# ElusAegis/metal-msm-gpu-acceleration

Hardware: AMD Instinct MI355X
Metric: BN254 G1 MSM/s at log_size=20 (5 instances) (higher is better)
Workload: dtype u32x8 (256-bit Montgomery integer)

## Files before the change

### include/msm_amd.h

```cpp
#ifndef MSM_AMD_H
#define MSM_AMD_H

#include <stddef.h>
#include <stdint.h>

#ifdef __cplusplus
extern "C" {
#endif

typedef struct msm_amd_ctx msm_amd_ctx;

enum {
  MSM_AMD_OK = 0,
  MSM_AMD_DEVICE_NOT_FOUND = 1,
  MSM_AMD_LIBRARY_ERROR = 2,
  MSM_AMD_FUNCTION_ERROR = 3,
  MSM_AMD_PIPELINE_ERROR = 4,
  MSM_AMD_INPUT_ERROR = 5,
  MSM_AMD_FILE_OPEN_ERROR = 6,
  MSM_AMD_DESERIALIZATION_ERROR = 7,
  MSM_AMD_INVALID_DATA = 8
};

enum {
// ... 150 lines not shown
size_t msm_amd_instances_default_path(const char* dir, uint32_t log_size, uint32_t num_instances, char* buf,
                                      size_t buf_len);
int msm_amd_to_wire(int scalar_layout, int point_layout, const void* scalars, const void* points, size_t n,
                    void* scalars_be32_out, void* points_be32_out);
int msm_amd_from_wire(int scalar_layout, int point_layout, const void* scalars_be32, const void* points_be32,
                      size_t n, void* scalars_out, void* points_out);

int msm_amd_prepare_buckets_indices(msm_amd_ctx* ctx, const uint32_t* scalars_be32, size_t n, uint32_t window_size,
                                    uint32_t num_windows, uint32_t* pairs_out);
int msm_amd_sort_buckets_indices(msm_amd_ctx* ctx, uint32_t* pairs, size_t n_pairs);
int msm_amd_sort_pairs_device(msm_amd_ctx* ctx, void* d_pairs, size_t n_pairs, uint32_t key_bits, float* kernel_ms);
int msm_amd_bucket_wise_accumulation(msm_amd_ctx* ctx, const uint32_t* sorted_pairs, size_t n_pairs,
                                     const uint32_t* points_be32, size_t n_points, uint32_t total_buckets,
                                     uint32_t* buckets_out);
int msm_amd_sum_reduction(msm_amd_ctx* ctx, const uint32_t* buckets_be32, uint32_t buckets_size,
                          uint32_t num_windows, uint32_t* res_out);
int msm_amd_final_accumulation(const uint32_t* res_be32, uint32_t num_windows, uint32_t window_size,
                               uint32_t* point_out);

enum {
  MSM_AMD_OP_UINT_ADD = 0,
  MSM_AMD_OP_UINT_SUB = 1,
  MSM_AMD_OP_UINT_PROD = 2,
  MSM_AMD_OP_UINT_SHL = 3,
  MSM_AMD_OP_UINT_SHR = 4,
  MSM_AMD_OP_FP_ADD = 5,
  MSM_AMD_OP_FP_SUB = 6,
  MSM_AMD_OP_FP_MUL = 7,
  MSM_AMD_OP_FP_NEG = 8,
  MSM_AMD_OP_FP_POW = 9,
  MSM_AMD_OP_EC_ADD = 10,
  MSM_AMD_OP_EC_MUL = 11,
  MSM_AMD_OP_EC_MADD = 12,
  MSM_AMD_OP_EC_DBL = 13,
  MSM_AMD_OP_FP29_MUL = 14,
  MSM_AMD_OP_FP29_SQR = 15,
  MSM_AMD_OP_FP29_SUB_K4E30 = 16,
  MSM_AMD_OP_FP29_SUB_K8E30 = 17,
  MSM_AMD_OP_FP29_SUB_K8E31 = 18,
  MSM_AMD_OP_FP29_SUB_K16E30 = 19,
  MSM_AMD_OP_FP29_SUB_K16E31 = 20,
  MSM_AMD_OP_FP29_ROUNDTRIP = 21,
  MSM_AMD_OP_EC29_MADD = 22,
  MSM_AMD_OP_EC29_ADD = 23,
  MSM_AMD_OP_EC29_MADD_CHAIN = 24,
  MSM_AMD_OP_EC29_ADD_CHAIN = 25,
  MSM_AMD_OP_EC29_MMADD = 26,
  MSM_AMD_OP_H64_FP_MUL = 27,
  MSM_AMD_OP_H64_FP_ADD = 28,
  MSM_AMD_OP_H64_FP_SUB = 29,
  MSM_AMD_OP_H64_EC_ADD = 30,
  MSM_AMD_OP_H64_EC_DBL = 31,
  MSM_AMD_OP_FP29_MUL_KARATSUBA = 32,
  MSM_AMD_OP_FP29_LOCKSTEP_PAIR = 33,
  MSM_AMD_OP_FP29_LOCKSTEP_MIX = 34,
  MSM_AMD_OP_FP29_LOCKSTEP_TRIPLE = 35,
  MSM_AMD_OP_FP29_MUL2_KARATSUBA = 36,
  MSM_AMD_OP_H64_FP_INV = 37,
  MSM_AMD_OP_H64_FP_INV_FERMAT = 38
};
int msm_amd_test_op(msm_amd_ctx* ctx, int op, const uint32_t* a, const uint32_t* b, uint32_t* out, size_t count);
int msm_amd_test_op_host(int op, const uint32_t* a, const uint32_t* b, uint32_t* out, size_t count);

enum {
  MSM_AMD_RAW_FE_MUL = 0,
  MSM_AMD_RAW_FE_SQR = 1,
  MSM_AMD_RAW_FE_MUL2 = 2,
  MSM_AMD_RAW_FE_SUB_K4E30 = 3,
  MSM_AMD_RAW_FE_SUB_K8E30 = 4,
  MSM_AMD_RAW_FE_SUB_K8E31 = 5,
  MSM_AMD_RAW_FE_SUB_K16E30 = 6,
  MSM_AMD_RAW_FE_SUB_K16E31 = 7,
  MSM_AMD_RAW_FE_NORM = 8,
  MSM_AMD_RAW_FE_NEG = 9,
  MSM_AMD_RAW_FE_NEG_WIDE = 10,
  MSM_AMD_RAW_FE_CANONICAL = 11,
  MSM_AMD_RAW_FE_TO_EXT = 12,
  MSM_AMD_RAW_FE_PACK_UNPACK = 13,
  MSM_AMD_RAW_FE_ZERO = 14,
  MSM_AMD_RAW_PT_MADD = 15,
  MSM_AMD_RAW_PT_MMADD = 16,
  MSM_AMD_RAW_PT_ADD_NZ = 17,
  MSM_AMD_RAW_PT_ADD = 18,
  MSM_AMD_RAW_PT_DOUBLE = 19
};
int msm_amd_test_op_raw(msm_amd_ctx* ctx, int op, const uint32_t* a, const uint32_t* b, uint32_t* out, size_t count);
int msm_amd_test_op_raw_host(int op, const uint32_t* a, const uint32_t* b, uint32_t* out, size_t count);

int msm_amd_test_hold(msm_amd_ctx* ctx, uint32_t max_ms, void** handle);
int msm_amd_test_release(msm_amd_ctx* ctx, void* handle);

enum {
  MSM_AMD_TP_C = 0, MSM_AMD_TP_W, MSM_AMD_TP_W_DIGITS, MSM_AMD_TP_N, MSM_AMD_TP_N_SCALARS, MSM_AMD_TP_LB, MSM_AMD_TP_NB,
  MSM_AMD_TP_CH, MSM_AMD_TP_HB, MSM_AMD_TP_MB, MSM_AMD_TP_FB, MSM_AMD_TP_Q, MSM_AMD_TP_TILED, MSM_AMD_TP_BALLOT,
  MSM_AMD_TP_WIDE_DIGITS, MSM_AMD_TP_LONE,
  MSM_AMD_TP_TOTAL_ITEMS, MSM_AMD_TP_MULTI_COUNT, MSM_AMD_TP_DEFERRED,
  MSM_AMD_TP_RED_GROUP, MSM_AMD_TP_RB_THREADS, MSM_AMD_TP_INSTANCES, MSM_AMD_TP_WORKSPACE, MSM_AMD_TP_FRONT_THREADS,
  MSM_AMD_TEST_PLAN_WORDS
};
int msm_amd_test_last_plan(msm_amd_ctx* ctx, uint32_t j, uint32_t* out, size_t count);
enum {
  MSM_AMD_STAGE_DIGITS = 0,
  MSM_AMD_STAGE_SORTED = 1,
  MSM_AMD_STAGE_BUCKET_SIZE = 2,
  MSM_AMD_STAGE_BUCKET_START = 3,
  MSM_AMD_STAGE_ITEM_START = 4,
  MSM_AMD_STAGE_WIN_ITEMS = 5,
  MSM_AMD_STAGE_ORDER = 6,
  MSM_AMD_STAGE_MULTI_LIST = 7,
  MSM_AMD_STAGE_BUCKETS = 8,
  MSM_AMD_STAGE_PARTIAL = 9
};
int msm_amd_test_stage_copy(msm_amd_ctx* ctx, uint32_t j, int which, void* out, size_t* bytes);
int msm_amd_test_fill_workspaces(msm_amd_ctx* ctx, uint8_t byte);

int msm_amd_last_timings(const msm_amd_ctx* ctx, msm_amd_timings* out);
uint64_t msm_amd_algorithmic_bytes(size_t n, uint32_t window_size, int accumulate_only);
const char* msm_amd_version(void);

#ifdef __cplusplus
}
#endif
#endif
```

### metal-msm-gpu-acceleration_amd/__init__.py

```python
from __future__ import annotations

import ctypes
import os
from ctypes import POINTER, c_char_p, c_float, c_int, c_size_t, c_uint32, c_uint64, c_void_p

_HERE = os.path.dirname(os.path.abspath(__file__))
LIB_PATH = os.environ.get("MSM_AMD_LIB") or os.path.join(_HERE, "libmsm_amd.so")

(OK, DEVICE_NOT_FOUND, LIBRARY_ERROR, FUNCTION_ERROR, PIPELINE_ERROR, INPUT_ERROR, FILE_OPEN_ERROR,
 DESERIALIZATION_ERROR, INVALID_DATA) = range(9)
SCALAR_MONT_LE, SCALAR_CANON_LE, SCALAR_CANON_BE32 = 0, 1, 2
POINT_H2C_AFFINE, POINT_ARK_PROJECTIVE, POINT_ARK_AFFINE, POINT_JAC_BE32, POINT_PREPARED, POINT_TABLES = 0, 1, 2, 3, 4, 5
POINT_BYTES = {POINT_H2C_AFFINE: 64, POINT_ARK_PROJECTIVE: 96, POINT_ARK_AFFINE: 72, POINT_JAC_BE32: 96}
(OP_UINT_ADD, OP_UINT_SUB, OP_UINT_PROD, OP_UINT_SHL, OP_UINT_SHR, OP_FP_ADD, OP_FP_SUB, OP_FP_MUL, OP_FP_NEG,
 OP_FP_POW, OP_EC_ADD, OP_EC_MUL, OP_EC_MADD, OP_EC_DBL, OP_FP29_MUL, OP_FP29_SQR, OP_FP29_SUB_K4E30,
 OP_FP29_SUB_K8E30, OP_FP29_SUB_K8E31, OP_FP29_SUB_K16E30, OP_FP29_SUB_K16E31, OP_FP29_ROUNDTRIP, OP_EC29_MADD,
 OP_EC29_ADD, OP_EC29_MADD_CHAIN, OP_EC29_ADD_CHAIN, OP_EC29_MMADD, OP_H64_FP_MUL, OP_H64_FP_ADD, OP_H64_FP_SUB,
 OP_H64_EC_ADD, OP_H64_EC_DBL, OP_FP29_MUL_KARATSUBA, OP_FP29_LOCKSTEP_PAIR, OP_FP29_LOCKSTEP_MIX,
 OP_FP29_LOCKSTEP_TRIPLE, OP_FP29_MUL2_KARATSUBA, OP_H64_FP_INV, OP_H64_FP_INV_FERMAT) = range(39)
(RAW_FE_MUL, RAW_FE_SQR, RAW_FE_MUL2, RAW_FE_SUB_K4E30, RAW_FE_SUB_K8E30, RAW_FE_SUB_K8E31, RAW_FE_SUB_K16E30,
 RAW_FE_SUB_K16E31, RAW_FE_NORM, RAW_FE_NEG, RAW_FE_NEG_WIDE, RAW_FE_CANONICAL, RAW_FE_TO_EXT, RAW_FE_PACK_UNPACK,
 RAW_FE_ZERO, RAW_PT_MADD, RAW_PT_MMADD, RAW_PT_ADD_NZ, RAW_PT_ADD, RAW_PT_DOUBLE) = range(20)
RAW_IN_WORDS, RAW_OUT_WORDS = 36, 40


def op_is_point(op):
    return 10 <= op <= 13 or 22 <= op <= 26 or op in (OP_H64_EC_ADD, OP_H64_EC_DBL)

EXPORTS = [
    "msm_amd_init", "msm_amd_init_reusable", "msm_amd_get_global", "msm_amd_destroy", "msm_amd_strerror",
    "msm_amd_last_error", "msm_amd_set_window_size", "msm_amd_auto_window_size", "msm_amd_auto_window_size_lone", "msm_amd_gpu_msm_h2c",
    "msm_amd_gpu_msm_h2c_sync", "msm_amd_cpu_dispatch_below", "msm_amd_host_register", "msm_amd_host_unregister",
    "msm_amd_metal_msm_ark", "msm_amd_msm", "msm_amd_msm_batch", "msm_amd_msm_best", "msm_amd_gpu_with_cpu",
    "msm_amd_reference_split", "msm_amd_msm_device",
    "msm_amd_msm_batch_device", "msm_amd_submit_batch_device", "msm_amd_wait_batch", "msm_amd_device_alloc", "msm_amd_device_free", "msm_amd_copy_to_device",
    "msm_amd_copy_to_host", "msm_amd_stream", "msm_amd_synchronize", "msm_amd_generate_instance",
    "msm_amd_prepare_buckets_indices", "msm_amd_sort_buckets_indices", "msm_amd_bucket_wise_accumulation",
    "msm_amd_sum_reduction", "msm_amd_final_accumulation", "msm_amd_test_op", "msm_amd_test_op_host",
    "msm_amd_test_op_raw", "msm_amd_test_op_raw_host",
    "msm_amd_last_timings",
    "msm_amd_algorithmic_bytes", "msm_amd_version",
    "msm_amd_instances_save", "msm_amd_instances_open", "msm_amd_instances_count", "msm_amd_instances_size",
    "msm_amd_instances_read", "msm_amd_instances_close", "msm_amd_instances_default_path", "msm_amd_to_wire",
    "msm_amd_from_wire", "msm_amd_sort_pairs_device", "msm_amd_bases_upload", "msm_amd_bases_prepare_device",
    "msm_amd_msm_prepared", "msm_amd_sum_points", "msm_amd_tables_build", "msm_amd_tables_build_device",
    "msm_amd_tables_info", "msm_amd_tables_free", "msm_amd_msm_tables",
    "msm_amd_set_wait_timeout_ms", "msm_amd_set_bases_cache", "msm_amd_bases_cache_stats", "msm_amd_test_hold",
    "msm_amd_test_release", "msm_amd_msm_batch_multi", "msm_amd_msm_batch_multi_device", "msm_amd_msm_range_multi", "msm_amd_shard_range",
    "msm_amd_submit_batch_multi_device", "msm_amd_wait_batch_multi", "msm_amd_bases_cache_invalidate",
    "msm_amd_set_bases_cache_verify",
    "msm_amd_scalar_bytes", "msm_amd_point_bytes", "msm_amd_shard_owner",
    "msm_amd_shard_count", "msm_amd_ctx_device", "msm_amd_pin_thread_to_device", "msm_amd_gather_init",
    "msm_amd_gather_size", "msm_amd_gather_all", "msm_amd_gather_last_error", "msm_amd_gather_destroy",
    "msm_amd_host_msm", "msm_amd_tuned_split", "msm_amd_host_threads", "msm_amd_generate_instance_host", "msm_amd_test_op_ifma",
    "msm_amd_test_last_plan", "msm_amd_test_stage_copy", "msm_amd_test_fill_workspaces",
]

TEST_PLAN_FIELDS = ("c", "W", "W_digits", "n", "n_scalars", "lb", "nb", "CH", "hb", "mb", "fb", "Q", "tiled", "ballot",
                    "wide_digits", "lone", "total_items", "multi_count", "deferred", "red_group", "rb_threads",
                    "instances", "workspace", "front_threads")
(STAGE_DIGITS, STAGE_SORTED, STAGE_BUCKET_SIZE, STAGE_BUCKET_START, STAGE_ITEM_START, STAGE_WIN_ITEMS, STAGE_ORDER,
 STAGE_MULTI_LIST, STAGE_BUCKETS, STAGE_PARTIAL) = range(10)


AFTER_SORT_FN = ctypes.CFUNCTYPE(None, c_void_p)


class Timings(ctypes.Structure):
    _fields_ = [("convert_ms", c_float), ("digits_ms", c_float), ("sort_ms", c_float), ("accumulate_ms", c_float),
                ("reduce_ms", c_float), ("final_ms", c_float), ("total_gpu_ms", c_float), ("n", c_uint32),
                ("window_size", c_uint32), ("num_windows", c_uint32), ("reserved", c_uint32),
                ("accumulate_kernel_ms", c_float), ("reserved2", c_float * 3)]


class MsmError(RuntimeError):

    def __init__(self, status, detail=""):
        self.status = status
        super().__init__(f"msm_amd status {status}: {_lib().msm_amd_strerror(status).decode()} {detail}")


_LIB = None


def _lib():
    global _LIB
    if _LIB is None:
        if not os.path.exists(LIB_PATH):
            raise FileNotFoundError(f"{LIB_PATH} not built: run `python -c 'import __graft_entry__ as g; g.build()'`")
        L = ctypes.CDLL(LIB_PATH)
        L.msm_amd_strerror.restype = c_char_p
        L.msm_amd_strerror.argtypes = [c_int]
        L.msm_amd_last_error.restype = c_char_p
        L.msm_amd_last_error.argtypes = [c_void_p]
        L.msm_amd_version.restype = c_char_p
        L.msm_amd_init.argtypes = [c_int, POINTER(c_void_p)]
        L.msm_amd_bases_upload.argtypes = [c_void_p, c_int, c_void_p, c_size_t, POINTER(c_void_p)]
        L.msm_amd_bases_prepare_device.argtypes = [c_void_p, c_int, c_void_p, c_size_t, c_void_p]
        L.msm_amd_msm_prepared.argtypes = [c_void_p, c_int, c_void_p, c_void_p, c_size_t, c_void_p]
        L.msm_amd_tables_build.argtypes = [c_void_p, c_int, c_void_p, c_size_t, c_uint32, POINTER(c_void_p)]
        L.msm_amd_tables_build_device.argtypes = [c_void_p, c_int, c_void_p, c_size_t, c_uint32, POINTER(c_void_p)]
        L.msm_amd_tables_info.argtypes = [c_void_p, c_void_p, POINTER(c_size_t), POINTER(c_uint32), POINTER(c_uint32),
                                          POINTER(c_size_t)]
        L.msm_amd_tables_free.argtypes = [c_void_p, c_void_p]
        L.msm_amd_msm_tables.argtypes = [c_void_p, c_void_p, c_int, c_void_p, c_void_p]
# ... 580 lines not shown
```

### metal-msm-gpu-acceleration_amd/csrc/bn254_ec29.hip.h

```cpp
#pragma once
#include "bn254_ec.hip.h"
#include "bn254_fq29.hip.h"

namespace msm_amd {

struct AffI {
  fe29 x, y;
};
struct AffPacked {
  u256 x, y;
};
struct PtI {
  fe29 x, y, zz, zzz;
};
static_assert(sizeof(AffPacked) == 64, "AffPacked must be 64 bytes");
static_assert(sizeof(PtI) == 144, "PtI must be 144 bytes");

MSM_HD bool affi_is_identity(const AffI& p) {
  uint32_t o = 0;
  MSM_UNROLL for (int i = 0; i < 9; ++i) o |= p.x.l[i] | p.y.l[i];
  return o == 0;
}
MSM_HD bool pti_is_identity(const PtI& p) { return Fq29::is_zero_limbs(p.zz); }

// ... 149 lines not shown
  const fe29 Pp = pin_limbs(P), Rp = pin_limbs(R), X1 = pin_limbs(px), Y1 = pin_limbs(py);
  const fe29 PP = Fq29::sqr_np(Pp);
  const fe29 PPP = Fq29::mul_np(Pp, PP);
  const fe29 Q = Fq29::mul_np(X1, PP);
  const fe29 RR = Fq29::sqr_np(Rp);
  PtI r;
  r.x = Fq29::norm(Fq29::sub<K8E31>(RR, Fq29::add(PPP, Fq29::add(Q, Q))));
  const fe29 T = Fq29::norm(Fq29::sub<K16E30>(Q, r.x));
  r.y = Fq29::mul2_np(Rp, T, Y1, Fq29::neg_wide(PPP));
  r.zz = PP;
  r.zzz = PPP;
  return r;
}

MSM_HD PtI pti_madd(const PtI& p, const AffI& q, bool& vanished) {
#if defined(MSM_AMD_EXPERIMENTS) && defined(MSM_FQ29_LOCKSTEP)
  fe29 U2, S2;
  Fq29::mul_pair(q.x, p.zz, q.y, p.zzz, U2, S2);
#elif defined(MSM_AMD_EXPERIMENTS) && defined(MSM_FQ29_KARATSUBA)
  const fe29 U2 = Fq29::mul_karatsuba(q.x, p.zz);
  const fe29 S2 = Fq29::mul_karatsuba(q.y, p.zzz);
#else
  fe29 U2, S2;
  PtI pp = p;
  pti_madd_head(pp, q.x, q.y, U2, S2);
  return pti_madd_tail(pp, U2, S2, [&]() { return q; }, vanished);
#endif
#if defined(MSM_AMD_EXPERIMENTS) && (defined(MSM_FQ29_LOCKSTEP) || defined(MSM_FQ29_KARATSUBA))
  const fe29 P = Fq29::norm(Fq29::sub<K16E30>(U2, p.x));
  const fe29 R = Fq29::norm(Fq29::sub<K8E30>(S2, p.y));
  if (Fq29::maybe_zero(P, 18)) {
    MSM_ISA_MARK("rare mixed_addition");
    if (Fq29::is_zero_exact(P)) {
      if (Fq29::is_zero_exact(R)) return pti_double(pti_from_affi(q));
      vanished = true;
      return pti_identity();
    }
  }
  MSM_ISA_MARK("resume mixed_addition");
  PtI r;
#if defined(MSM_AMD_EXPERIMENTS) && defined(MSM_FQ29_LOCKSTEP)
  fe29 PP, RR, PPP, Q;
  Fq29::sqr_pair(P, R, PP, RR);
  Fq29::mul_triple(P, PP, p.x, PP, p.zz, PP, PPP, Q, r.zz);
  r.x = Fq29::norm(Fq29::sub<K8E31>(RR, Fq29::add(PPP, Fq29::add(Q, Q))));
  const fe29 T = Fq29::sub<K16E30>(Q, r.x);
  Fq29::mul2_mul_pair(R, T, p.y, Fq29::neg_wide(PPP), p.zzz, PPP, r.y, r.zzz);
#elif defined(MSM_AMD_EXPERIMENTS) && defined(MSM_FQ29_KARATSUBA)
  const fe29 PP = Fq29::sqr(P);
  const fe29 PPP = Fq29::mul_karatsuba(P, PP);
  const fe29 Q = Fq29::mul_karatsuba(p.x, PP);
  const fe29 RR = Fq29::sqr(R);
  r.x = Fq29::norm(Fq29::sub<K8E31>(RR, Fq29::add(PPP, Fq29::add(Q, Q))));
  const fe29 T = Fq29::sub<K16E30>(Q, r.x);
  r.y = Fq29::mul2_karatsuba_second(R, T, p.y, Fq29::neg_wide(PPP));
  r.zz = Fq29::mul_karatsuba(p.zz, PP);
  r.zzz = Fq29::mul_karatsuba(p.zzz, PPP);
#endif
  return r;
#endif
}

MSM_HD PtI pti_mmadd(const fe29& px, const fe29& py, const AffI& q, bool& vanished) {
  fe29 P, R;
  pti_mmadd_head(px, py, q.x, q.y, P, R);
  return pti_mmadd_tail(px, py, P, R, [&]() { return q; }, vanished);
}


#if defined(MSM_AMD_EXPERIMENTS)
#include "experiments/ec29_variants.inc"
#endif

MSM_HD PtI pti_madd(const PtI& p, const AffI& q) {
  bool vanished = false;
  return pti_madd(p, q, vanished);
}
MSM_HD PtI pti_mmadd(const fe29& px, const fe29& py, const AffI& q) {
  bool vanished = false;
  return pti_mmadd(px, py, q, vanished);
}

MSM_HD PtI pti_add_nz(const PtI& p_in, const PtI& q_in, bool& vanished) {
  PtI p, q;
  p.x = pin_limbs(p_in.x); p.y = pin_limbs(p_in.y); p.zz = pin_limbs(p_in.zz); p.zzz = pin_limbs(p_in.zzz);
  q.x = pin_limbs(q_in.x); q.y = pin_limbs(q_in.y); q.zz = pin_limbs(q_in.zz); q.zzz = pin_limbs(q_in.zzz);
  const fe29 U1a = Fq29::mul_np(p.x, q.zz);
  const fe29 U2 = Fq29::mul_np(q.x, p.zz);
  const fe29 S1a = Fq29::mul_np(p.y, q.zzz);
  const fe29 S2 = Fq29::mul_np(q.y, p.zzz);
  const fe29 P0 = Fq29::norm(Fq29::sub<K4E30>(U2, U1a));
  const fe29 R0 = Fq29::norm(Fq29::sub<K4E30>(S2, S1a));
  if (Fq29::maybe_zero(P0, 6)) {
    if (Fq29::is_zero_exact(P0)) {
      if (Fq29::is_zero_exact(R0)) return pti_double(p);
      vanished = true;
      return pti_identity();
    }
  }
  const fe29 P = pin_limbs(P0), R = pin_limbs(R0), U1 = pin_limbs(U1a), S1 = pin_limbs(S1a), ZZ1 = pin_limbs(p.zz),
             ZZ2 = pin_limbs(q.zz), ZZZ1 = pin_limbs(p.zzz), ZZZ2 = pin_limbs(q.zzz);
  const fe29 PP = Fq29::sqr_np(P);
  const fe29 PPP = Fq29::mul_np(P, PP);
  const fe29 Q = Fq29::mul_np(U1, PP);
  const fe29 RR = Fq29::sqr_np(R);
  PtI r;
  r.x = Fq29::norm(Fq29::sub<K8E31>(RR, Fq29::add(PPP, Fq29::add(Q, Q))));
  const fe29 T = Fq29::sub<K16E30>(Q, r.x);
  r.y = Fq29::mul2_np(R, T, S1, Fq29::neg_wide(PPP));
  r.zz = Fq29::mul_np(Fq29::mul_np(ZZ1, ZZ2), PP);
  r.zzz = Fq29::mul_np(Fq29::mul_np(ZZZ1, ZZZ2), PPP);
  return r;
}
MSM_HD PtI pti_add_nz(const PtI& p, const PtI& q) {
  bool vanished = false;
  return pti_add_nz(p, q, vanished);
}

MSM_HD PtI pti_add(const PtI& p, const PtI& q) {
  if (pti_is_identity(p)) return q;
  if (pti_is_identity(q)) return p;
  return pti_add_nz(p, q);
}

}
```

### metal-msm-gpu-acceleration_amd/csrc/bn254_fq29.hip.h

```cpp
#pragma once
#include "bn254_fq.hip.h"

namespace msm_amd {

struct fe29 {
  uint32_t l[9];
};

MSM_HD uint32_t limb32(uint32_t x) {
#if defined(__HIP_DEVICE_COMPILE__) && !defined(MSM_FQ29_NOPIN)
  asm("" : "+v"(x));
#endif
  return x;
}
MSM_HD fe29 pin_limbs(const fe29& a) {
  fe29 r;
#if defined(__HIP_DEVICE_COMPILE__)
  _Pragma("unroll") for (int i = 0; i < 9; ++i) r.l[i] = limb32(a.l[i]);
#else
  r = a;
#endif
  return r;
}

#if defined(__HIP_DEVICE_COMPILE__)
#define MSM_ISA_MARK(name) asm volatile("; MSM_MARK " name)
#else
#define MSM_ISA_MARK(name) ((void)0)
#endif

enum KSel { K4E30 = 0, K8E30 = 1, K8E31 = 2, K16E30 = 3, K16E31 = 4 };

struct Fq29 {
  static constexpr uint32_t MASK = 0x1FFFFFFFu;
  static constexpr uint32_t INV = 0x04866389u;
  static constexpr uint32_t PINV = 0x1B799C77u;

  MSM_HD static constexpr uint32_t p(int i) {
    constexpr uint32_t c[9] = {0x187CFD47u, 0x010460B6u, 0x1C72A34Fu, 0x02D522D0u, 0x1585D978u,
                               0x02DB40C0u, 0x00A6E141u, 0x0E5C2634u, 0x0030644Eu};
    return c[i];
  }
  MSM_HD static constexpr uint32_t one_c(int i) {
    constexpr uint32_t c[9] = {0x157CCC21u, 0x141C2758u, 0x185230D3u, 0x014C0419u, 0x0AA36FB9u,
                               0x1D4240CEu, 0x11D54C07u, 0x052AC7A8u, 0x000DC836u};
    return c[i];
  }
  MSM_HD static constexpr uint32_t cin_c(int i) {
    constexpr uint32_t c[9] = {0x13349CA1u, 0x1A5D84A8u, 0x0A3E5CACu, 0x100249E0u, 0x12B951E8u,
                               0x0E92D304u, 0x14CB95B3u, 0x041B9D3Du, 0x00058003u};
    return c[i];
  }
  MSM_HD static constexpr uint32_t dout_c(int i) {
    constexpr uint32_t c[9] = {0x058F0D9Du, 0x1AEA1C6Eu, 0x11C2CF74u, 0x11D651EBu, 0x1462C0A7u,
                               0x11B7BC3Cu, 0x1CBD99BAu, 0x183340FBu, 0x000E0A77u};
    return c[i];
  }
  MSM_HD static constexpr uint32_t kc(int sel, int i) {
    constexpr uint32_t c[5][9] = {
        {0x41F3F51Cu, 0x441182D9u, 0x51CA8D3Au, 0x4B548B41u, 0x561765DEu, 0x4B6D0300u, 0x429B8502u, 0x597098CEu, 0x00C19137u},
        {0x43E7EA38u, 0x482305B4u, 0x43951A76u, 0x56A91685u, 0x4C2ECBBEu, 0x56DA0603u, 0x45370A06u, 0x52E1319Eu, 0x01832271u},
        {0x83E7EA38u, 0x882305B2u, 0x83951A74u, 0x96A91683u, 0x8C2ECBBCu, 0x96DA0601u, 0x85370A04u, 0x92E1319Cu, 0x0183226Fu},
        {0x47CFD470u, 0x50460B6Au, 0x472A34EEu, 0x4D522D0Cu, 0x585D977Fu, 0x4DB40C08u, 0x4A6E140Fu, 0x45C2633Eu, 0x030644E5u},
        {0x87CFD470u, 0x90460B68u, 0x872A34ECu, 0x8D522D0Au, 0x985D977Du, 0x8DB40C06u, 0x8A6E140Du, 0x85C2633Cu, 0x030644E3u}};
    return c[sel][i];
  }

  MSM_HD static fe29 zero() {
    fe29 r;
    MSM_UNROLL for (int i = 0; i < 9; ++i) r.l[i] = 0;
    return r;
  }
  MSM_HD static fe29 one() {
    fe29 r;
    MSM_UNROLL for (int i = 0; i < 9; ++i) r.l[i] = one_c(i);
    return r;
  }
  MSM_HD static bool is_zero_limbs(const fe29& a) {
    uint32_t o = 0;
    MSM_UNROLL for (int i = 0; i < 9; ++i) o |= a.l[i];
    return o == 0;
  }

  MSM_HD static fe29 add(const fe29& a, const fe29& b) {
    fe29 r;
    MSM_UNROLL for (int i = 0; i < 9; ++i) r.l[i] = a.l[i] + b.l[i];
    return r;
  }

  template <int SEL>
  MSM_HD static fe29 sub(const fe29& a, const fe29& b) {
    fe29 r;
    MSM_UNROLL for (int i = 0; i < 9; ++i) r.l[i] = (a.l[i] + kc(SEL, i)) - b.l[i];
    return r;
  }

  MSM_HD static fe29 neg(const fe29& a) { return norm(sub<K4E30>(zero(), a)); }
  MSM_HD static fe29 neg_wide(const fe29& a) { return sub<K4E30>(zero(), a); }

  MSM_HD static fe29 norm(const fe29& a) {
    fe29 r;
    r.l[0] = a.l[0] & MASK;
    MSM_UNROLL for (int i = 1; i < 8; ++i) r.l[i] = (a.l[i] & MASK) + (a.l[i - 1] >> 29);
    r.l[8] = a.l[8] + (a.l[7] >> 29);
    return r;
  }

  MSM_HD static fe29 reduce_columns(uint64_t (&A)[17]) {
    uint64_t carry = 0;
    MSM_UNROLL for (int k = 0; k < 9; ++k) {
      A[k] += carry;
      const uint32_t m = ((uint32_t)A[k] * INV) & MASK;
      MSM_UNROLL for (int j = 0; j < 9; ++j) A[k + j] += (uint64_t)m * p(j);
      carry = A[k] >> 29;
    }
    fe29 r;
    MSM_UNROLL for (int k = 9; k < 17; ++k) {
      A[k] += carry;
      r.l[k - 9] = (uint32_t)A[k] & MASK;
      carry = A[k] >> 29;
    }
    r.l[8] = (uint32_t)carry;
    return r;
  }


#if defined(MSM_AMD_EXPERIMENTS)
#include "experiments/fq29_variants.inc"
#endif

  template <bool PIN = true>
  MSM_HD static fe29 mul(const fe29& a_in, const fe29& b_in) {
    const fe29 a = PIN ? pin_limbs(a_in) : a_in, b = PIN ? pin_limbs(b_in) : b_in;
#if defined(MSM_AMD_EXPERIMENTS) && defined(MSM_FQ29_FIPS)
    {
      const fe29* const xs[1] = {&a};
      const fe29* const ys[1] = {&b};
      return fips<1>(xs, ys);
    }
#endif
    uint64_t A[17];
    MSM_UNROLL for (int k = 0; k < 17; ++k) {
      uint64_t s = 0;
      MSM_UNROLL for (int i = 0; i < 9; ++i) {
        const int j = k - i;
        if (j >= 0 && j < 9) s += (uint64_t)a.l[i] * b.l[j];
      }
      A[k] = s;
    }
    return reduce_columns(A);
  }

  template <bool PIN = true>
  MSM_HD static fe29 mul2(const fe29& a_in, const fe29& b_in, const fe29& c_in, const fe29& d_in) {
    const fe29 a = PIN ? pin_limbs(a_in) : a_in, b = PIN ? pin_limbs(b_in) : b_in, c = PIN ? pin_limbs(c_in) : c_in,
               d = PIN ? pin_limbs(d_in) : d_in;
#if defined(MSM_AMD_EXPERIMENTS) && defined(MSM_FQ29_FIPS)
    {
      const fe29* const xs[2] = {&a, &c};
      const fe29* const ys[2] = {&b, &d};
      return fips<2>(xs, ys);
    }
#endif
    uint64_t A[17];
    MSM_UNROLL for (int k = 0; k < 17; ++k) {
      uint64_t s = 0;
      MSM_UNROLL for (int i = 0; i < 9; ++i) {
        const int j = k - i;
        if (j >= 0 && j < 9) {
          s += (uint64_t)a.l[i] * b.l[j];
          s += (uint64_t)c.l[i] * d.l[j];
        }
      }
      A[k] = s;
    }
    return reduce_columns(A);
  }

  template <bool PIN = true>
  MSM_HD static fe29 sqr(const fe29& a_in) {
    const fe29 a = PIN ? pin_limbs(a_in) : a_in;
#if defined(MSM_AMD_EXPERIMENTS) && defined(MSM_FQ29_FIPS)
    {
      fe29 d2;
      MSM_UNROLL for (int i = 0; i < 9; ++i) d2.l[i] = a.l[i] << 1;
      const fe29* const xs[1] = {&d2};
      const fe29* const ys[1] = {&a};
      return fips<1, true>(xs, ys);
    }
#endif
    uint32_t d[9];
    MSM_UNROLL for (int i = 0; i < 9; ++i) d[i] = a.l[i] << 1;
    uint64_t A[17];
    MSM_UNROLL for (int k = 0; k < 17; ++k) {
      uint64_t s = 0;
      MSM_UNROLL for (int i = 0; i < 9; ++i) {
        const int j = k - i;
        if (j >= 0 && j < 9 && i < j) s += (uint64_t)d[i] * a.l[j];
      }
      if ((k & 1) == 0) s += (uint64_t)a.l[k >> 1] * a.l[k >> 1];
      A[k] = s;
    }
    return reduce_columns(A);
  }
  MSM_HD static fe29 mul_np(const fe29& a, const fe29& b) { return mul<false>(a, b); }
  MSM_HD static fe29 sqr_np(const fe29& a) { return sqr<false>(a); }
  MSM_HD static fe29 mul2_np(const fe29& a, const fe29& b, const fe29& c, const fe29& d) { return mul2<false>(a, b, c, d); }

  MSM_HD static fe29 unpack256(const u256& x) {
    fe29 t;
    MSM_UNROLL for (int i = 0; i < 9; ++i) {
      const int bit = 29 * i;
      const int w = bit >> 5, s = bit & 31;
      uint32_t v = x.v[w] >> s;
      if (s > 3 && w + 1 < 8) v |= x.v[w + 1] << (32 - s);
      t.l[i] = (i < 8) ? (v & MASK) : v;
    }
    return t;
  }

  MSM_HD static u256 pack256(const fe29& t) {
    u256 r;
    MSM_UNROLL for (int w = 0; w < 8; ++w) {
      const int bit = 32 * w;
      const int i = bit / 29, s = bit % 29;
      uint32_t v = t.l[i] >> s;
      if (i + 1 < 9) v |= t.l[i + 1] << (29 - s);
      if (29 - s + 29 < 32 && i + 2 < 9) v |= t.l[i + 2] << (58 - s);
      r.v[w] = v;
    }
    return r;
  }

  MSM_HD static fe29 from_ext(const u256& x) {
    fe29 c;
    MSM_UNROLL for (int i = 0; i < 9; ++i) c.l[i] = cin_c(i);
    return mul(unpack256(x), c);
  }

  MSM_HD static fe29 canonical(const fe29& a, int rounds) {
    fe29 r;
    uint32_t carry = 0;
    MSM_UNROLL for (int i = 0; i < 8; ++i) {
      const uint64_t s = (uint64_t)a.l[i] + carry;
      r.l[i] = (uint32_t)s & MASK;
      carry = (uint32_t)(s >> 29);
    }
    r.l[8] = a.l[8] + carry;
    for (int it = 0; it < rounds; ++it) {
      fe29 d;
      int32_t borrow = 0;
      MSM_UNROLL for (int i = 0; i < 9; ++i) {
        const int32_t s = (int32_t)r.l[i] - (int32_t)p(i) + borrow;
        d.l[i] = (i < 8) ? ((uint32_t)s & MASK) : (uint32_t)s;
        borrow = (i < 8) ? (s >> 29) : 0;
        if (i == 8) borrow = (s < 0) ? -1 : 0;
      }
      if (borrow == 0) r = d;
    }
    return r;
  }

  MSM_HD static u256 to_ext(const fe29& a) {
    fe29 d;
    MSM_UNROLL for (int i = 0; i < 9; ++i) d.l[i] = dout_c(i);
    return pack256(canonical(mul(a, d), 1));
  }

  MSM_HD static u256 pack_canonical(const fe29& a) { return pack256(canonical(a, 1)); }

  MSM_HD static bool maybe_zero(const fe29& a, uint32_t bound) {
    return (((a.l[0] & MASK) * PINV) & MASK) < bound;
  }

  MSM_HD static bool is_zero_exact(const fe29& a) {
    const fe29 t = canonical(mul(a, one()), 1);
    return is_zero_limbs(t);
  }
};

}
```

### metal-msm-gpu-acceleration_amd/csrc/msm_host.hip

```cpp
#include <hip/hip_runtime.h>

#include <algorithm>
#include <atomic>
#include <chrono>
#include <cmath>
#include <cstdio>
#include <cstdlib>
#include <cstring>
#include <condition_variable>
#include <mutex>
#include <string>
#include <thread>
#include <vector>

#include "../../include/msm_amd.h"
#include "device_common.hip.h"
#include "launch.h"
#include "host_fq64.h"
#include "test_ops.hip.h"

using namespace msm_amd;

namespace {

// ... 2460 lines not shown
    for (uint32_t i = 0; i < window_size; ++i) acc = h64::jdouble(acc);
    acc = h64::jadd(acc, h64::load(be32_to_jac(res_be32 + (size_t)w * 24)));
  }
  jac_to_be32(h64::store(acc), point_out);
  return MSM_AMD_OK;
}

static void test_op_widths(int op, size_t* wa, size_t* wb) {
  const bool pt = test_op_is_point(op);
  *wa = pt ? 3 : 1;
  *wb = (op == MSM_AMD_OP_EC_MUL) ? 1 : *wa;
}

int msm_amd_test_op(msm_amd_ctx* ctx, int op, const uint32_t* a, const uint32_t* b, uint32_t* out, size_t count) {
  if (!ctx || !a || !b || !out || count == 0 || op < 0 || op > kTestOpMax ||
      (op >= MSM_AMD_OP_H64_FP_MUL && op <= MSM_AMD_OP_H64_EC_DBL))
    return fail(ctx, MSM_AMD_INPUT_ERROR, "bad test_op arguments");
  std::lock_guard<std::mutex> g(ctx->mu);
  HIP_TRY(ctx, hipSetDevice(ctx->device));
  hipStream_t st = ctx->stream;
  size_t wa, wb;
  test_op_widths(op, &wa, &wb);
  const size_t wo = wa;
  std::vector<uint32_t> la(count * wa * 8), lb(count * wb * 8), lo(count * wo * 8);
  for (size_t i = 0; i < count * wa; ++i)
    for (int l = 0; l < 8; ++l) la[i * 8 + l] = a[i * 8 + 7 - l];
  for (size_t i = 0; i < count * wb; ++i)
    for (int l = 0; l < 8; ++l) lb[i * 8 + l] = b[i * 8 + 7 - l];
  int rc;
  if ((rc = ensure(ctx, ctx->scratch_a, la.size() * 4))) return rc;
  if ((rc = ensure(ctx, ctx->scratch_b, lb.size() * 4))) return rc;
  if ((rc = ensure(ctx, ctx->scratch_c, lo.size() * 4))) return rc;
  HIP_TRY(ctx, hipMemcpyAsync(ctx->scratch_a.p, la.data(), la.size() * 4, hipMemcpyHostToDevice, st));
  HIP_TRY(ctx, hipMemcpyAsync(ctx->scratch_b.p, lb.data(), lb.size() * 4, hipMemcpyHostToDevice, st));
  launch_test_op(st, op, (const u256*)ctx->scratch_a.p, (const u256*)ctx->scratch_b.p, (u256*)ctx->scratch_c.p,
                 (uint32_t)count);
  HIP_TRY(ctx, hipGetLastError());
  HIP_TRY(ctx, hipMemcpyAsync(lo.data(), ctx->scratch_c.p, lo.size() * 4, hipMemcpyDeviceToHost, st));
  if (int src_ = sync_stream_bounded(ctx, st, __func__)) return src_;
  for (size_t i = 0; i < count * wo; ++i)
    for (int l = 0; l < 8; ++l) out[i * 8 + l] = lo[i * 8 + 7 - l];
  return MSM_AMD_OK;
}

static bool host64_test_op(int op, const uint32_t* a, const uint32_t* b, uint32_t* out, size_t count) {
  const bool inverse = op == MSM_AMD_OP_H64_FP_INV || op == MSM_AMD_OP_H64_FP_INV_FERMAT;
  if ((op < MSM_AMD_OP_H64_FP_MUL || op > MSM_AMD_OP_H64_EC_DBL) && !inverse) return false;
  const bool pt = op == MSM_AMD_OP_H64_EC_ADD || op == MSM_AMD_OP_H64_EC_DBL;
  for (size_t t = 0; t < count; ++t) {
    if (!pt) {
      const u256 xa = be32_to_u256(a + t * 8), xb = be32_to_u256(b + t * 8);
      h64::Fe x, y, r;
      std::memcpy(&x, &xa, 32);
      std::memcpy(&y, &xb, 32);
      if (inverse) r = op == MSM_AMD_OP_H64_FP_INV ? h64::inv(x) : h64::inv_fermat(x);
      else r = op == MSM_AMD_OP_H64_FP_MUL ? h64::mul(x, y) : (op == MSM_AMD_OP_H64_FP_ADD ? h64::add(x, y) : h64::sub(x, y));
      u256 ro;
      std::memcpy(&ro, &r, 32);
      u256_to_be32(ro, out + t * 8);
    } else {
      const h64::Jac p = h64::load(be32_to_jac(a + t * 24)), q = h64::load(be32_to_jac(b + t * 24));
      jac_to_be32(h64::store(op == MSM_AMD_OP_H64_EC_ADD ? h64::jadd(p, q) : h64::jdouble(p)), out + t * 24);
    }
  }
  return true;
}

int msm_amd_test_op_host(int op, const uint32_t* a, const uint32_t* b, uint32_t* out, size_t count) {
  if (!a || !b || !out || count == 0 || op < 0) return MSM_AMD_INPUT_ERROR;
  if (host64_test_op(op, a, b, out, count)) return MSM_AMD_OK;
  if (op > kTestOpMax) return MSM_AMD_INPUT_ERROR;
  size_t wa, wb;
  test_op_widths(op, &wa, &wb);
  const size_t wo = wa;
  std::vector<u256> la(count * wa), lb(count * std::max(wb, wa)), lo(count * wo);
  for (size_t i = 0; i < count * wa; ++i) la[i] = be32_to_u256(a + i * 8);
  for (size_t i = 0; i < count * wb; ++i) lb[i] = be32_to_u256(b + i * 8);
  for (size_t t = 0; t < count; ++t) run_test_op(op, la.data(), lb.data(), lo.data(), (uint32_t)t);
  for (size_t i = 0; i < count * wo; ++i) u256_to_be32(lo[i], out + i * 8);
  return MSM_AMD_OK;
}

static bool test_op_raw_args(int op, const uint32_t* a, const uint32_t* b, uint32_t* out, size_t count) {
  return a && b && out && count > 0 && count <= (1u << 24) && op >= 0 && op < kRawOpCount;
}

int msm_amd_test_op_raw(msm_amd_ctx* ctx, int op, const uint32_t* a, const uint32_t* b, uint32_t* out, size_t count) {
  if (!ctx || !test_op_raw_args(op, a, b, out, count)) return fail(ctx, MSM_AMD_INPUT_ERROR, "bad test_op_raw arguments");
  std::lock_guard<std::mutex> g(ctx->mu);
  HIP_TRY(ctx, hipSetDevice(ctx->device));
  hipStream_t st = ctx->stream;
  const size_t in_bytes = count * kRawInWords * 4, out_bytes = count * kRawOutWords * 4;
  int rc;
  if ((rc = ensure(ctx, ctx->scratch_a, in_bytes))) return rc;
  if ((rc = ensure(ctx, ctx->scratch_b, in_bytes))) return rc;
  if ((rc = ensure(ctx, ctx->scratch_c, out_bytes))) return rc;
  HIP_TRY(ctx, hipMemcpyAsync(ctx->scratch_a.p, a, in_bytes, hipMemcpyHostToDevice, st));
  HIP_TRY(ctx, hipMemcpyAsync(ctx->scratch_b.p, b, in_bytes, hipMemcpyHostToDevice, st));
  launch_test_op_raw(st, op, (const uint32_t*)ctx->scratch_a.p, (const uint32_t*)ctx->scratch_b.p,
                     (uint32_t*)ctx->scratch_c.p, (uint32_t)count);
  HIP_TRY(ctx, hipGetLastError());
  HIP_TRY(ctx, hipMemcpyAsync(out, ctx->scratch_c.p, out_bytes, hipMemcpyDeviceToHost, st));
  return sync_stream_bounded(ctx, st, __func__);
}

int msm_amd_test_op_raw_host(int op, const uint32_t* a, const uint32_t* b, uint32_t* out, size_t count) {
  if (!test_op_raw_args(op, a, b, out, count)) return MSM_AMD_INPUT_ERROR;
  for (size_t t = 0; t < count; ++t) run_test_op_raw(op, a, b, out, (uint32_t)t);
  return MSM_AMD_OK;
}

int msm_amd_test_hold(msm_amd_ctx* ctx, uint32_t max_ms, void** handle) {
  if (!ctx || !handle || max_ms == 0 || max_ms > 5000) return fail(ctx, MSM_AMD_INPUT_ERROR, "bad test_hold arguments");
  std::lock_guard<std::mutex> g(ctx->mu);
  HIP_TRY(ctx, hipSetDevice(ctx->device));
  uint32_t* flag = nullptr;
  HIP_TRY(ctx, hipHostMalloc((void**)&flag, 64, hipHostMallocDefault));
  *flag = 0;
  launch_hold(ctx->stream, flag, (uint64_t)max_ms * 100000ull);
  const hipError_t e = hipGetLastError();
  if (e != hipSuccess) {
    (void)hipHostFree(flag);
    HIP_TRY(ctx, e);
  }
  *handle = flag;
  return MSM_AMD_OK;
}

int msm_amd_test_release(msm_amd_ctx* ctx, void* handle) {
  if (!ctx || !handle) return MSM_AMD_INPUT_ERROR;
  std::lock_guard<std::mutex> g(ctx->mu);
  HIP_TRY(ctx, hipSetDevice(ctx->device));
  *(volatile uint32_t*)handle = 1u;
  HIP_TRY(ctx, hipStreamSynchronize(ctx->stream));
  HIP_TRY(ctx, hipHostFree(handle));
  return MSM_AMD_OK;
}

static int tap_batch(msm_amd_ctx* ctx, uint32_t j, const Batch** out) {
  if (ctx->last_waited < 0) return fail(ctx, MSM_AMD_INPUT_ERROR, "stage tap: no batch has been waited for");
  const Batch& B = ctx->batches[ctx->last_waited];
  if (B.active || B.n_inst > (size_t)kWorkspaces || B.ws_index.size() != B.n_inst)
    return fail(ctx, MSM_AMD_INPUT_ERROR, "stage tap: the last batch had more instances than the ctx has workspaces");
  if (j >= B.n_inst) return fail(ctx, MSM_AMD_INPUT_ERROR, "stage tap: no such instance in the last batch");
  *out = &B;
  return MSM_AMD_OK;
}

int msm_amd_test_last_plan(msm_amd_ctx* ctx, uint32_t j, uint32_t* out, size_t count) {
  if (!ctx || !out || count < MSM_AMD_TEST_PLAN_WORDS) return fail(ctx, MSM_AMD_INPUT_ERROR, "bad test_last_plan arguments");
  std::lock_guard<std::mutex> g(ctx->mu);
  const Batch* B = nullptr;
  if (int rc = tap_batch(ctx, j, &B)) return rc;
  const Plan& p = B->plans[j];
  const InstanceSlot& s = B->slots[j];
  PlanCounters pc;
  std::memcpy(&pc, s.h_partial + s.h_partial_cap, sizeof pc);
  uint32_t v[MSM_AMD_TEST_PLAN_WORDS] = {};
  v[MSM_AMD_TP_C] = p.c;
  v[MSM_AMD_TP_W] = p.W;
  v[MSM_AMD_TP_W_DIGITS] = p.W_digits;
  v[MSM_AMD_TP_N] = p.n;
  v[MSM_AMD_TP_N_SCALARS] = p.n_scalars;
  v[MSM_AMD_TP_LB] = p.lb;
  v[MSM_AMD_TP_NB] = p.nb;
  v[MSM_AMD_TP_CH] = p.CH;
  v[MSM_AMD_TP_HB] = p.hb;
// ... 113 lines not shown
```

Baseline: 801.3.

## Use wide Montgomery reduction and fused mul2 in full point addition

Restructures the full Jacobian-ZZ point addition so P and R are each computed with a single fused dual-product (mul2) instead of two separate multiplications followed by a subtraction. The later formulas are reordered so ZZ2·PP and ZZZ2·PPP are reused for Q, the y-coordinate and the output zz/zzz. It also adds a 'wide' reduction mode that skips masking the Montgomery quotient for the lower limbs, saving an AND per step, and makes it the default for mul_np and sqr_np. The trade-off is that outputs become less reduced, which means looser limb bounds for later ops (the maybe-zero check bound changes accordingly), with a correctness risk if downstream code assumed tighter bounds.

```diff
diff --git a/include/msm_amd.h b/include/msm_amd.h
--- a/include/msm_amd.h
+++ b/include/msm_amd.h
@@ -256,7 +256,10 @@
   MSM_AMD_RAW_PT_MMADD = 16,
   MSM_AMD_RAW_PT_ADD_NZ = 17,
   MSM_AMD_RAW_PT_ADD = 18,
-  MSM_AMD_RAW_PT_DOUBLE = 19
+  MSM_AMD_RAW_PT_DOUBLE = 19,
+  MSM_AMD_RAW_FE_MUL_WIDE = 32,
+  MSM_AMD_RAW_FE_SQR_WIDE = 33,
+  MSM_AMD_RAW_FE_MUL2_WIDE = 34
 };
 int msm_amd_test_op_raw(msm_amd_ctx* ctx, int op, const uint32_t* a, const uint32_t* b, uint32_t* out, size_t count);
 int msm_amd_test_op_raw_host(int op, const uint32_t* a, const uint32_t* b, uint32_t* out, size_t count);
diff --git a/metal-msm-gpu-acceleration_amd/__init__.py b/metal-msm-gpu-acceleration_amd/__init__.py
--- a/metal-msm-gpu-acceleration_amd/__init__.py
+++ b/metal-msm-gpu-acceleration_amd/__init__.py
@@ -21,6 +21,7 @@
 (RAW_FE_MUL, RAW_FE_SQR, RAW_FE_MUL2, RAW_FE_SUB_K4E30, RAW_FE_SUB_K8E30, RAW_FE_SUB_K8E31, RAW_FE_SUB_K16E30,
  RAW_FE_SUB_K16E31, RAW_FE_NORM, RAW_FE_NEG, RAW_FE_NEG_WIDE, RAW_FE_CANONICAL, RAW_FE_TO_EXT, RAW_FE_PACK_UNPACK,
  RAW_FE_ZERO, RAW_PT_MADD, RAW_PT_MMADD, RAW_PT_ADD_NZ, RAW_PT_ADD, RAW_PT_DOUBLE) = range(20)
+RAW_FE_MUL_WIDE, RAW_FE_SQR_WIDE, RAW_FE_MUL2_WIDE = range(32, 35)
 RAW_IN_WORDS, RAW_OUT_WORDS = 36, 40
 
 
diff --git a/metal-msm-gpu-acceleration_amd/csrc/bn254_ec29.hip.h b/metal-msm-gpu-acceleration_amd/csrc/bn254_ec29.hip.h
--- a/metal-msm-gpu-acceleration_amd/csrc/bn254_ec29.hip.h
+++ b/metal-msm-gpu-acceleration_amd/csrc/bn254_ec29.hip.h
@@ -255,34 +255,36 @@
 }
 
 MSM_HD PtI pti_add_nz(const PtI& p_in, const PtI& q_in, bool& vanished) {
+  MSM_ISA_MARK("begin full_addition");
   PtI p, q;
   p.x = pin_limbs(p_in.x); p.y = pin_limbs(p_in.y); p.zz = pin_limbs(p_in.zz); p.zzz = pin_limbs(p_in.zzz);
   q.x = pin_limbs(q_in.x); q.y = pin_limbs(q_in.y); q.zz = pin_limbs(q_in.zz); q.zzz = pin_limbs(q_in.zzz);
-  const fe29 U1a = Fq29::mul_np(p.x, q.zz);
-  const fe29 U2 = Fq29::mul_np(q.x, p.zz);
-  const fe29 S1a = Fq29::mul_np(p.y, q.zzz);
-  const fe29 S2 = Fq29::mul_np(q.y, p.zzz);
-  const fe29 P0 = Fq29::norm(Fq29::sub<K4E30>(U2, U1a));
-  const fe29 R0 = Fq29::norm(Fq29::sub<K4E30>(S2, S1a));
-  if (Fq29::maybe_zero(P0, 6)) {
+  const fe29 P0 = Fq29::mul2w_np(q.x, p.zz, p.x, Fq29::neg_wide(q.zz));
+  const fe29 R0 = Fq29::mul2w_np(q.y, p.zzz, p.y, Fq29::neg_wide(q.zzz));
+  if (Fq29::maybe_zero(P0, 2)) {
+    MSM_ISA_MARK("rare full_addition");
     if (Fq29::is_zero_exact(P0)) {
       if (Fq29::is_zero_exact(R0)) return pti_double(p);
       vanished = true;
       return pti_identity();
     }
   }
-  const fe29 P = pin_limbs(P0), R = pin_limbs(R0), U1 = pin_limbs(U1a), S1 = pin_limbs(S1a), ZZ1 = pin_limbs(p.zz),
+  MSM_ISA_MARK("resume full_addition");
+  const fe29 P = pin_limbs(P0), R = pin_limbs(R0), X1 = pin_limbs(p.x), Y1 = pin_limbs(p.y), ZZ1 = pin_limbs(p.zz),
              ZZ2 = pin_limbs(q.zz), ZZZ1 = pin_limbs(p.zzz), ZZZ2 = pin_limbs(q.zzz);
   const fe29 PP = Fq29::sqr_np(P);
   const fe29 PPP = Fq29::mul_np(P, PP);
-  const fe29 Q = Fq29::mul_np(U1, PP);
+  const fe29 V = Fq29::mul_np(ZZ2, PP);
+  const fe29 Tz = Fq29::mul_np(ZZZ2, PPP);
+  const fe29 Q = Fq29::mul_np(X1, V);
   const fe29 RR = Fq29::sqr_np(R);
   PtI r;
   r.x = Fq29::norm(Fq29::sub<K8E31>(RR, Fq29::add(PPP, Fq29::add(Q, Q))));
   const fe29 T = Fq29::sub<K16E30>(Q, r.x);
-  r.y = Fq29::mul2_np(R, T, S1, Fq29::neg_wide(PPP));
-  r.zz = Fq29::mul_np(Fq29::mul_np(ZZ1, ZZ2), PP);
-  r.zzz = Fq29::mul_np(Fq29::mul_np(ZZZ1, ZZZ2), PPP);
+  r.y = Fq29::mul2_np(R, T, Y1, Fq29::neg_wide(Tz));
+  r.zz = Fq29::mul_np(ZZ1, V);
+  r.zzz = Fq29::mul_np(ZZZ1, Tz);
+  MSM_ISA_MARK("end full_addition");
   return r;
 }
 MSM_HD PtI pti_add_nz(const PtI& p, const PtI& q) {
diff --git a/metal-msm-gpu-acceleration_amd/csrc/bn254_fq29.hip.h b/metal-msm-gpu-acceleration_amd/csrc/bn254_fq29.hip.h
--- a/metal-msm-gpu-acceleration_amd/csrc/bn254_fq29.hip.h
+++ b/metal-msm-gpu-acceleration_amd/csrc/bn254_fq29.hip.h
@@ -106,11 +106,12 @@
     return r;
   }
 
+  template <bool WIDE = false>
   MSM_HD static fe29 reduce_columns(uint64_t (&A)[17]) {
     uint64_t carry = 0;
     MSM_UNROLL for (int k = 0; k < 9; ++k) {
       A[k] += carry;
-      const uint32_t m = ((uint32_t)A[k] * INV) & MASK;
+      const uint32_t m = (WIDE && k < 8) ? (uint32_t)A[k] * INV : ((uint32_t)A[k] * INV) & MASK;
       MSM_UNROLL for (int j = 0; j < 9; ++j) A[k + j] += (uint64_t)m * p(j);
       carry = A[k] >> 29;
     }
@@ -129,7 +130,7 @@
 #include "experiments/fq29_variants.inc"
 #endif
 
-  template <bool PIN = true>
+  template <bool PIN = true, bool WIDE = false>
   MSM_HD static fe29 mul(const fe29& a_in, const fe29& b_in) {
     const fe29 a = PIN ? pin_limbs(a_in) : a_in, b = PIN ? pin_limbs(b_in) : b_in;
 #if defined(MSM_AMD_EXPERIMENTS) && defined(MSM_FQ29_FIPS)
@@ -148,10 +149,10 @@
       }
       A[k] = s;
     }
-    return reduce_columns(A);
-  }
-
-  template <bool PIN = true>
+    return reduce_columns<WIDE>(A);
+  }
+
+  template <bool PIN = true, bool WIDE = false>
   MSM_HD static fe29 mul2(const fe29& a_in, const fe29& b_in, const fe29& c_in, const fe29& d_in) {
     const fe29 a = PIN ? pin_limbs(a_in) : a_in, b = PIN ? pin_limbs(b_in) : b_in, c = PIN ? pin_limbs(c_in) : c_in,
                d = PIN ? pin_limbs(d_in) : d_in;
@@ -174,10 +175,10 @@
       }
       A[k] = s;
     }
-    return reduce_columns(A);
-  }
-
-  template <bool PIN = true>
+    return reduce_columns<WIDE>(A);
+  }
+
+  template <bool PIN = true, bool WIDE = false>
   MSM_HD static fe29 sqr(const fe29& a_in) {
     const fe29 a = PIN ? pin_limbs(a_in) : a_in;
 #if defined(MSM_AMD_EXPERIMENTS) && defined(MSM_FQ29_FIPS)
@@ -201,11 +202,14 @@
       if ((k & 1) == 0) s += (uint64_t)a.l[k >> 1] * a.l[k >> 1];
       A[k] = s;
     }
-    return reduce_columns(A);
-  }
-  MSM_HD static fe29 mul_np(const fe29& a, const fe29& b) { return mul<false>(a, b); }
-  MSM_HD static fe29 sqr_np(const fe29& a) { return sqr<false>(a); }
+    return reduce_columns<WIDE>(A);
+  }
+  MSM_HD static fe29 mul_np(const fe29& a, const fe29& b) { return mul<false, true>(a, b); }
+  MSM_HD static fe29 sqr_np(const fe29& a) { return sqr<false, true>(a); }
   MSM_HD static fe29 mul2_np(const fe29& a, const fe29& b, const fe29& c, const fe29& d) { return mul2<false>(a, b, c, d); }
+  MSM_HD static fe29 mul2w_np(const fe29& a, const fe29& b, const fe29& c, const fe29& d) {
+    return mul2<false, true>(a, b, c, d);
+  }
 
   MSM_HD static fe29 unpack256(const u256& x) {
     fe29 t;
diff --git a/metal-msm-gpu-acceleration_amd/csrc/msm_host.hip b/metal-msm-gpu-acceleration_amd/csrc/msm_host.hip
--- a/metal-msm-gpu-acceleration_amd/csrc/msm_host.hip
+++ b/metal-msm-gpu-acceleration_amd/csrc/msm_host.hip
@@ -2566,7 +2566,8 @@
 }
 
 static bool test_op_raw_args(int op, const uint32_t* a, const uint32_t* b, uint32_t* out, size_t count) {
-  return a && b && out && count > 0 && count <= (1u << 24) && op >= 0 && op < kRawOpCount;
+  return a && b && out && count > 0 && count <= (1u << 24) && op >= 0 &&
+         (op < kRawOpCount || (op >= kRawWideFirst && op < kRawWideFirst + kRawWideCount));
 }
 
 int msm_amd_test_op_raw(msm_amd_ctx* ctx, int op, const uint32_t* a, const uint32_t* b, uint32_t* out, size_t count) {
```

New measurement: 822.2 (median of 6 runs). 1.03x the previous value.
